# kthohr/mcmc

Hardware: AMD Instinct MI355X
Metric: leapfrog-steps/sec (chains*dims*steps/s), HMC d=128 correlated Gaussian, 65536 chains (higher is better)
Workload: dtype f64

## Files before the change

include/mi_mcmc_engine/det_math.hpp:

```cpp
#pragma once

#include <hip/hip_runtime.h>
#include <stdint.h>

#define MI_HD __host__ __device__ __forceinline__

#if defined(__HIP_DEVICE_COMPILE__)
#define MI_NO_DS_MERGE __attribute__((target("no-load-store-opt")))
#else
#define MI_NO_DS_MERGE
#endif

namespace mi {

#ifndef MI_KC_MODE
#define MI_KC_MODE 1
#endif
#if defined(__HIP_DEVICE_COMPILE__) && MI_KC_MODE == 1
__device__ __forceinline__ double mi_kc(double c) { asm volatile("" : "+s"(c)); return c; }
#define MI_KC(c) ::mi::mi_kc(c)
#define MI_KCD(c, dep) ::mi::mi_kc(c)
#elif defined(__HIP_DEVICE_COMPILE__) && MI_KC_MODE == 2
template <uint64_t BITS>
__device__ __forceinline__ double mi_kc()
{
    uint32_t lo, hi;
    asm volatile("s_mov_b32 %0, %2\n\ts_mov_b32 %1, %3" : "=s"(lo), "=s"(hi) : "n"((uint32_t)BITS), "n"((uint32_t)(BITS >> 32)));
    return __builtin_bit_cast(double, ((uint64_t)hi << 32) | (uint64_t)lo);
}
template <uint64_t BITS>
__device__ __forceinline__ double mi_kcd(double dep)
{
    uint32_t lo, hi;
    asm volatile("s_mov_b32 %0, %2\n\ts_mov_b32 %1, %3" : "=s"(lo), "=s"(hi) : "n"((uint32_t)BITS), "n"((uint32_t)(BITS >> 32)), "v"(dep));
    return __builtin_bit_cast(double, ((uint64_t)hi << 32) | (uint64_t)lo);
}
#define MI_KC(c) (::mi::mi_kc<__builtin_bit_cast(uint64_t, (double)(c))>())
#define MI_KCD(c, dep) (::mi::mi_kcd<__builtin_bit_cast(uint64_t, (double)(c))>(dep))
#else
#define MI_KC(c) (c)
#define MI_KCD(c, dep) (c)
#endif


MI_HD uint64_t d2u(double x) { return __builtin_bit_cast(uint64_t, x); }
MI_HD double u2d(uint64_t u) { return __builtin_bit_cast(double, u); }
MI_HD double pow2i(int k) { return u2d((uint64_t)(k + 1023) << 52); }
MI_HD double dfma(double a, double b, double c) { return __builtin_fma(a, b, c); }
MI_HD bool is_finite(double x) { return (d2u(x) & 0x7ff0000000000000ULL) != 0x7ff0000000000000ULL; }

constexpr double LN2_HI = 0x1.62e42fee00000p-1;
constexpr double LN2_LO = 0x1.a39ef35793c76p-33;
constexpr double INV_LN2 = 0x1.71547652b82fep+0;
constexpr double PI_4 = 0x1.921fb54442d18p-1;
constexpr double INF = __builtin_huge_val();

MI_HD double det_exp(double x)
{
    if (x != x) return x;
    if (x > 709.782712893384) return INF;
    if (x < -745.2) return 0.0;
    const double kf = __builtin_rint(x * INV_LN2);
    const int k = (int)kf;
    double r = dfma(-kf, LN2_HI, x);
    r = dfma(-kf, LN2_LO, r);
    double p = MI_KCD(1.0 / 87178291200.0, r);
    p = dfma(p, r, MI_KCD(1.0 / 6227020800.0, p));
    p = dfma(p, r, MI_KCD(1.0 / 479001600.0, p));
    p = dfma(p, r, MI_KCD(1.0 / 39916800.0, p));
    p = dfma(p, r, MI_KCD(1.0 / 3628800.0, p));
    p = dfma(p, r, MI_KCD(1.0 / 362880.0, p));
    p = dfma(p, r, MI_KCD(1.0 / 40320.0, p));
    p = dfma(p, r, MI_KCD(1.0 / 5040.0, p));
    p = dfma(p, r, MI_KCD(1.0 / 720.0, p));
    p = dfma(p, r, MI_KCD(1.0 / 120.0, p));
    p = dfma(p, r, MI_KCD(1.0 / 24.0, p));
    p = dfma(p, r, MI_KCD(1.0 / 6.0, p));
    p = dfma(p, r, 0.5);
    p = dfma(p, r, 1.0);
    p = dfma(p, r, 1.0);
    const int k1 = k / 2, k2 = k - k1;
    return (p * pow2i(k1)) * pow2i(k2);
// ... 226 lines not shown
```

include/mi_mcmc_engine/hmc_dense.hpp:

```cpp
#pragma once

#include "det_math.hpp"

#ifndef MI_HMC_RNG_STAGED
#define MI_HMC_RNG_STAGED 0
#endif

#ifndef MI_HMC_RNG_PAIRS
#define MI_HMC_RNG_PAIRS 1
#endif

#ifndef MI_HMC_WPB
#define MI_HMC_WPB 8
#endif

namespace mi {

typedef double double4_t __attribute__((ext_vector_type(4)));

struct HmcParams {
    const double* P;
    uint32_t d;
    uint64_t C;
    uint64_t chain0;
// ... 190 lines not shown
            if (v != v) return (ub - lb) / 2;
            return (v < 0.0) ? lb + EPS_DBL : ub - EPS_DBL;
        }
        const double e = det_exp(v);
        const double r = (lb - EPS_DBL + (ub + EPS_DBL) * e) / (1.0 + e);
        return is_finite(r) ? r : ub - EPS_DBL;
    }
    default: return v;
    }
}
__device__ MI_BOX_INLINE double box_inv_jacobian(double v, int bt, double lb, double ub)
{
    switch (bt) {
    case 2: return det_exp(-v);
    case 3: return det_exp(v);
    case 4: { const double e = det_exp(v); return ((e + 1) * (e + 1)) / (e * (ub - lb)); }
    default: return 1.0;
    }
}
__device__ MI_BOX_INLINE double box_log_jacobian_term(double v, int bt, double lb, double ub)
{
    switch (bt) {
    case 2: return v;
    case 3: return -v;
    case 4: {
        const double e = det_exp(v);
        if (is_finite(e)) return det_log(ub - lb) + v - 2 * det_log(1 + e);
        return det_log(ub - lb) - v;
    }
    default: return 0.0;
    }
}

template <int NT, int WPB, bool BOUNDED = false, bool DENSE_M = false, bool DIAGM = false, bool PCM = false>
__global__ MI_NO_DS_MERGE __launch_bounds__(64 * WPB, WPB / 4) void hmc_gauss_mfma_kernel(const HmcParams prm)
{
    static_assert(!PCM || DIAGM, "per-chain masses ride the diagonal-mass variant");
    static_assert(!DENSE_M || BOUNDED, "the dense preconditioner rides the general variant");
    static_assert(!DIAGM || !BOUNDED, "DIAGM is the plain kernel with a diagonal mass; bounds take the general variant");
    constexpr int NS = 4 * NT;
    extern __shared__ __attribute__((aligned(16))) double lds_P[];
    stage_precision<NT>(prm.P, prm.d, lds_P);
    double* lds_lb = lds_P + NT * NS * 64;
    double* lds_ub = lds_lb + 16 * NT;
    double* lds_ms = lds_ub + 16 * NT;
    double* lds_mi = lds_ms + 16 * NT;
    int* lds_bt = reinterpret_cast<int*>(lds_mi + 16 * NT);
    double* lds_Minv = lds_mi + 16 * NT + 8 * NT;
    double* lds_L = lds_Minv + NT * NS * 64;
    if constexpr (DENSE_M && !dense_m_from_global<NT>()) {
        stage_precision<NT>(prm.Minv, prm.d, lds_Minv);
        stage_precision<NT>(prm.Lchol, prm.d, lds_L);
    }
    if (BOUNDED) {
        for (int i = threadIdx.x; i < 16 * NT; i += blockDim.x) {
            const bool in = (uint32_t)i < prm.d;
            lds_lb[i] = in ? prm.lb[i] : 0.0;
            lds_ub[i] = in ? prm.ub[i] : 0.0;
            lds_bt[i] = in ? prm.btype[i] : 1;
            lds_ms[i] = in ? prm.m_sqrt[i] : 1.0;
            lds_mi[i] = in ? prm.m_inv[i] : 1.0;
        }
        __syncthreads();
    }
    if (DIAGM && !PCM) {
        for (int i = threadIdx.x; i < 16 * NT; i += blockDim.x) {
            const bool in = (uint32_t)i < prm.d;
            lds_ms[i] = in ? prm.m_sqrt[i] : 1.0;
            lds_mi[i] = in ? prm.m_inv[i] : 1.0;
        }
        __syncthreads();
    }

    const int lane = threadIdx.x & 63, wave = threadIdx.x >> 6;
    const int j = lane >> 4;
    uint32_t bslices = 0;
    if constexpr (BOUNDED) {
        if (prm.vals_bound)
            for (int s_ = 0; s_ < 4 * NT; ++s_) {
                const bool any = lds_bt[4 * s_] != 1 || lds_bt[4 * s_ + 1] != 1 || lds_bt[4 * s_ + 2] != 1 || lds_bt[4 * s_ + 3] != 1;
                bslices |= (any ? 1u : 0u) << s_;
            }
        bslices = (uint32_t)__builtin_amdgcn_readfirstlane((int)bslices);
    }
    auto slice_bounded = [&](int s) -> bool { return ((bslices >> s) & 1u) != 0u; };
    [[maybe_unused]] auto mi_col = [&]() __attribute__((always_inline)) -> const double* {
        const double* p = lds_mi + (lane >> 4);
        asm volatile("" : "+v"(p));
        return p;
    };
    const uint64_t cl = ((uint64_t)blockIdx.x * WPB + wave) * 16 + (lane & 15);
    const bool live = cl < prm.C;
    const uint64_t cld = live ? cl : prm.C - 1;
    [[maybe_unused]] auto pcm_at = [&](const double* tab, int s) __attribute__((always_inline)) -> double {
        uint32_t dim = 4u * (uint32_t)s + (uint32_t)(lane >> 4);
        asm volatile("" : "+v"(dim));
        return tab[(size_t)(dim < prm.d ? dim : 0u) * prm.C + cld];
    };
    auto minv_at = [&]([[maybe_unused]] const double* mic, int s) __attribute__((always_inline)) -> double {
        if constexpr (PCM) return pcm_at(prm.m_inv, s); else return mic[4 * s];
    };
    const uint64_t chain = prm.chain0 + cl;
    const uint32_t d = prm.d;
    const uint64_t C = prm.C;
    const double eps = prm.eps;
    const double* afrag = lds_P + lane;
    [[maybe_unused]] const double* afrag_minv = (DENSE_M && dense_m_from_global<NT>()) ? prm.Minv + lane : lds_Minv + lane;
    [[maybe_unused]] const double* afrag_l = (DENSE_M && dense_m_from_global<NT>()) ? prm.Lchol + lane : lds_L + lane;

    double th[NS], pm[NS], w[NS];
    double xs[BOUNDED ? NS : 1];
    const size_t lane_off = (size_t)j * C + cld;
    double* const ws_wave = prm.wsave + ((size_t)blockIdx.x * WPB + wave) * ((size_t)3 * NS * 64) + lane;
    auto ws_group = [&](int k) -> double* {
        double* b = ws_wave + (size_t)(k & ~7) * 64;
        asm volatile("" : "+v"(b));
        return b + (k & 7) * 64;
    };
    auto th_mem = [&](int s) -> double* { return ws_group(s); };
    auto w_mem = [&](int s) -> double* { return ws_group(NS + s); };
    [[maybe_unused]] auto z_mem = [&](int s) -> double* { return ws_wave + (size_t)(2 * NS + s) * 64; };

    auto gradient = [&]() __attribute__((always_inline)) {
        if constexpr (BOUNDED) {
#pragma unroll
            for (int s = 0; s < NS; ++s) {
                const int i = 4 * s + j;
                if (slice_bounded(s)) xs[s] = ((uint32_t)i < d) ? box_inv_transform(th[s], lds_bt[i], lds_lb[i], lds_ub[i]) : 0.0;
                else xs[s] = ((uint32_t)i < d) ? th[s] : 0.0;
            }
            target_times<NT>(afrag, prm.P, d, prm.sep_target != 0u, xs, w);
        } else {
            matvec_mfma<NT>(afrag, th, w);
        }
    };
    auto kick_terms = [&](double (&t)[BOUNDED ? NS : 1]) __attribute__((always_inline)) {
        if constexpr (BOUNDED) {
#pragma unroll
            for (int s = 0; s < NS; ++s) {
                const int i = 4 * s + j;
                if (slice_bounded(s)) t[s] = box_inv_jacobian(th[s], lds_bt[i], lds_lb[i], lds_ub[i]) * w[s];
                else t[s] = 1.0 * w[s];
            }
            if (prm.vals_bound) dense_product_poison<NS>(w, t, j, d);
#pragma unroll
            for (int s = 0; s < NS; ++s) t[s] = (eps * t[s]) / 2.0;
        }
    };
    auto kinetic = [&]() __attribute__((always_inline)) -> double {
        if constexpr (BOUNDED) {
            double mp[NS];
            if constexpr (DENSE_M) {
                matvec_m2<NT>(afrag_minv, pm, mp);
            } else {
#pragma unroll
                for (int s = 0; s < NS; ++s) mp[s] = lds_mi[4 * s + j] * pm[s];
                dense_product_poison<NS>(pm, mp, j, d);
            }
            double q = 0.0;
#pragma unroll
            for (int s = 0; s < NS; ++s) q = dfma(pm[s], mp[s], q);
            q = q + __shfl_xor(q, 32);
            q = q + __shfl_xor(q, 16);
            return q / 2.0;
        } else if constexpr (DIAGM) {
            double q = 0.0;
            const double* mic = PCM ? nullptr : mi_col();
#pragma unroll
            for (int s = 0; s < NS; ++s) q = dfma(pm[s], minv_at(mic, s) * pm[s], q);
            q = q + __shfl_xor(q, 32);
            q = q + __shfl_xor(q, 16);
            return q / 2.0;
        } else {
            return dot4<NS>(pm, pm) / 2.0;
        }
    };
    auto potential = [&]() __attribute__((always_inline)) -> double {
        if constexpr (BOUNDED) {
            const double kval = -0.5 * dot4<NS>(xs, w);
            double lj = 0.0;
#pragma unroll
            for (int s = 0; s < NS; ++s) {
                if (!slice_bounded(s)) continue;
                const int i0 = 4 * s;
                const int bt = lds_bt[4 * s + j];
                const double term = box_log_jacobian_term(th[s], bt, lds_lb[4 * s + j], lds_ub[4 * s + j]);
#pragma unroll
                for (int g = 0; g < 4; ++g) {
                    const double tg = __shfl(term, (lane & 15) + 16 * g);
                    if ((uint32_t)(i0 + g) < d && lds_bt[i0 + g] != 1) lj = lj + tg;
                }
            }
            return -(kval + lj);
        } else {
            return 0.5 * dot4<NS>(th, w);
        }
    };

#pragma unroll
    for (int s = 0; s < NS; ++s) {
        const uint32_t dim = 4 * s + j;
        const double v = prm.theta[(size_t)(dim < d ? dim : 0u) * C + cld];
        if constexpr (BOUNDED) th[s] = (dim < d) ? box_transform(v, lds_bt[dim], lds_lb[dim], lds_ub[dim]) : 0.0;
        else th[s] = (dim < d) ? v : 0.0;
    }
    gradient();
    if (live) {
#pragma unroll
        for (int s = 0; s < NS; ++s) { *th_mem(s) = th[s]; *w_mem(s) = w[s]; }
    }
    double prev_U = potential();
    uint64_t n_acc = 0;
    const uint32_t n_total = prm.n_burnin + prm.n_keep;
    [[maybe_unused]] bool nf_seen = false;

    if (WPB > 4 && wave >= 4)
        for (uint32_t k = 0; k < prm.stagger; ++k) __builtin_amdgcn_s_sleep(127);

    const unsigned long long t_loop0 = clock64();
#pragma unroll 1
    for (uint32_t draw = 0; draw < n_total; ++draw) {
#if MI_HMC_RNG_STAGED
#pragma unroll 1
        for (int b = 0; b < NS / 2; ++b) {
            double z0, z1;
            if (prm.ablate & 4u) { z0 = 0.25; z1 = -0.5; }
            else rng_normal_pair_at(prm.seed, chain, draw + prm.draw0, (uint32_t)(4 * b), (uint32_t)j, STREAM_NORMAL, z0, z1);
            *z_mem(2 * b) = (8u * b + j < d) ? z0 : 0.0;
            *z_mem(2 * b + 1) = (8u * b + 4 + j < d) ? z1 : 0.0;
        }
#pragma unroll
        for (int s = 0; s < NS; ++s) pm[s] = *z_mem(s);
        if constexpr (DENSE_M) {
            double zz[NS];
#pragma unroll
            for (int s = 0; s < NS; ++s) zz[s] = pm[s];
            matvec_m2<NT>(afrag_l, zz, pm);
        } else if constexpr (BOUNDED || DIAGM) {
#pragma unroll
            for (int s = 0; s < NS; ++s) pm[s] = lds_ms[4 * s + j] * pm[s];
        }
#else
#pragma unroll
        for (int b = 0; b < NS / 2; ++b) {
            double z0, z1;
            if (prm.ablate & 4u) { z0 = 0.25; z1 = -0.5; }
            else rng_normal_pair_at(prm.seed, chain, draw + prm.draw0, (uint32_t)(4 * b), (uint32_t)j, STREAM_NORMAL, z0, z1);
            pm[2 * b] = (8u * b + j < d) ? z0 : 0.0;
            pm[2 * b + 1] = (8u * b + 4 + j < d) ? z1 : 0.0;
            if constexpr (DIAGM && PCM) {
                pm[2 * b] = pcm_at(prm.m_sqrt, 2 * b) * pm[2 * b];
                pm[2 * b + 1] = pcm_at(prm.m_sqrt, 2 * b + 1) * pm[2 * b + 1];
            } else if constexpr (DIAGM) {
                const double* msc = lds_ms + (lane >> 4);
                asm volatile("" : "+v"(msc));
                pm[2 * b] = msc[8 * b] * pm[2 * b];
                pm[2 * b + 1] = msc[8 * b + 4] * pm[2 * b + 1];
            } else if constexpr (BOUNDED && !DENSE_M) {
                pm[2 * b] = lds_ms[8 * b + j] * pm[2 * b];
                pm[2 * b + 1] = lds_ms[8 * b + 4 + j] * pm[2 * b + 1];
            }
            if (BOUNDED || MI_HMC_RNG_PAIRS == 1 || (b & 1)) __builtin_amdgcn_sched_barrier(0);
        }
        if constexpr (DENSE_M) {
            double zz[NS];
#pragma unroll
            for (int s = 0; s < NS; ++s) zz[s] = pm[s];
            matvec_m2<NT>(afrag_l, zz, pm);
        }
#endif
        const double prev_K = kinetic();

        if constexpr (!BOUNDED) {
            const uint32_t L = prm.n_leap_steps;
            if (L > 0 && (prm.ablate & 3u) != 1u) {
                [[maybe_unused]] const double* mic = (DIAGM && !PCM) ? mi_col() : nullptr;
#pragma unroll
                for (int s = 0; s < NS; ++s) {
                    pm[s] = pm[s] - (eps * w[s]) / 2.0;
                    if constexpr (DIAGM) th[s] = th[s] + eps * (minv_at(mic, s) * pm[s]);
                    else th[s] = th[s] + eps * pm[s];
                }
            }
#pragma unroll 1
            for (uint32_t k = 0; k + 1 < L; ++k) {
                if ((prm.ablate & 3u) != 2u) gradient();
                if ((prm.ablate & 3u) != 1u) {
                    [[maybe_unused]] const double* mic = (DIAGM && !PCM) ? mi_col() : nullptr;
#pragma unroll
                    for (int s = 0; s < NS; ++s) {
                        const double t = (eps * w[s]) / 2.0;
                        pm[s] = pm[s] - t;
                        pm[s] = pm[s] - t;
                        if constexpr (DIAGM) th[s] = th[s] + eps * (minv_at(mic, s) * pm[s]);
                        else th[s] = th[s] + eps * pm[s];
                    }
                }
            }
            if (L > 0) {
                if ((prm.ablate & 3u) != 2u) gradient();
                if ((prm.ablate & 3u) != 1u) {
#pragma unroll
                    for (int s = 0; s < NS; ++s) pm[s] = pm[s] - (eps * w[s]) / 2.0;
                }
            }
        } else {
            const uint32_t L = prm.n_leap_steps;
            auto drift_step = [&]() __attribute__((always_inline)) {
                double mp[NS];
                if constexpr (DENSE_M) {
                    matvec_m2<NT>(afrag_minv, pm, mp);
                } else {
#pragma unroll
                    for (int s = 0; s < NS; ++s) mp[s] = lds_mi[4 * s + j] * pm[s];
                    dense_product_poison<NS>(pm, mp, j, d);
                }
#pragma unroll
                for (int s = 0; s < NS; ++s) th[s] = th[s] + eps * mp[s];
            };
            if (L > 0) {
                double t[NS];
                kick_terms(t);
#pragma unroll
                for (int s = 0; s < NS; ++s) pm[s] = pm[s] - t[s];
                drift_step();
            }
#pragma unroll 1
            for (uint32_t k = 0; k + 1 < L; ++k) {
                gradient();
                double t[NS];
                kick_terms(t);
#pragma unroll
                for (int s = 0; s < NS; ++s) {
                    pm[s] = pm[s] - t[s];
                    pm[s] = pm[s] - t[s];
                }
                drift_step();
            }
            if (L > 0) {
                gradient();
                double t[NS];
                kick_terms(t);
#pragma unroll
                for (int s = 0; s < NS; ++s) pm[s] = pm[s] - t[s];
            }
        }
        if constexpr (BOUNDED) { if (prm.n_leap_steps == 0) gradient(); }

        double prop_U = potential();
        const bool u_nf = !is_finite(prop_U);
        if (u_nf) prop_U = INF;
        const double prop_K = kinetic();
        if constexpr (!BOUNDED) nf_seen |= u_nf | !is_finite(prop_K);
        const double x = -(prop_U + prop_K) + (prev_U + prev_K);
        const double comp_val = (x < 0.01) ? x : 0.01;
        const double z = rng_uniform(prm.seed, chain, draw + prm.draw0, 0u);
        const bool accept = z < det_exp(comp_val);
#ifndef MI_HMC_NO_WSAVE
#define MI_HMC_NO_WSAVE 0
#endif
        if constexpr (MI_HMC_NO_WSAVE && !BOUNDED) {
            if (accept) {
                prev_U = prop_U;
                if (live && !(prm.ablate & 8u)) {
#pragma unroll
                    for (int s = 0; s < NS; ++s) *th_mem(s) = th[s];
                }
            }
            if (__ballot(!accept) != 0ull) {
                if (!accept) {
#pragma unroll
                    for (int s = 0; s < NS; ++s) th[s] = *th_mem(s);
                }
                gradient();
            }
        } else
        if (accept) {
            prev_U = prop_U;
            if (live && !(prm.ablate & 8u)) {
#pragma unroll
                for (int s = 0; s < NS; ++s) { *th_mem(s) = th[s]; *w_mem(s) = w[s]; }
            }
        } else {
#pragma unroll
            for (int s = 0; s < NS; ++s) { th[s] = *th_mem(s); w[s] = *w_mem(s); }
        }
        if (draw >= prm.n_burnin) {
            n_acc += accept ? 1u : 0u;
            if (prm.draws != nullptr && live && !(prm.ablate & 16u)) {
                double* out = prm.draws + (size_t)(draw - prm.n_burnin) * d * C;
#pragma unroll
                for (int s = 0; s < NS; ++s) {
                    const uint32_t dim = 4 * s + j;
                    if (dim < d) (out + (size_t)(4 * s) * C)[lane_off] =
                        (BOUNDED && slice_bounded(s)) ? box_inv_transform(th[s], lds_bt[dim], lds_lb[dim], lds_ub[dim]) : th[s];
                }
            }
        }
    }

    bool replay = false;
    if constexpr (!BOUNDED) replay = nf_seen && prm.nf_flag != nullptr;
    if (live && replay && j == 0) { prm.nf_flag[cl] = 1u; prm.nf_flag[C] = 1u; }
    if (live && !replay) {
#pragma unroll
        for (int s = 0; s < NS; ++s) {
            const uint32_t dim = 4 * s + j;
            if (dim < d) prm.theta[(size_t)dim * C + cl] =
                (BOUNDED && slice_bounded(s)) ? box_inv_transform(th[s], lds_bt[dim], lds_lb[dim], lds_ub[dim]) : th[s];
        }
    }
    if (live && !replay && j == 0) {
        if (prm.n_accept) prm.n_accept[cl] = n_acc;
        if (prm.n_leap) prm.n_leap[cl] = (prm.ablate & 32u) ? (uint64_t)(clock64() - t_loop0)
                                                            : (uint64_t)n_total * prm.n_leap_steps;
    }
}

}
```

include/mi_mcmc_engine/tile_samplers.hpp:

```cpp
#pragma once

#include <type_traits>

#include "hmc_dense.hpp"

namespace mi {

struct TileParams {
    uint32_t d;
    uint64_t C, chain0;
    double* theta;
    double* wsave;
    double* draws;
    uint64_t* n_accept;
    uint64_t* n_leap;
    uint64_t seed;
    uint32_t n_burnin, n_keep, n_leap_steps, draw0;
    double eps;
    double s2, rs, cons_term, log_det;
    double* ws;
    double* step_out;
    uint32_t* depth_trace;
    double* adapt_state;
    uint32_t n_adapt, max_depth;
// ... 194 lines not shown
        const double v = prm.theta[(size_t)(dim < d ? dim : 0u) * C + cld];
        th[s] = (dim < d) ? v : 0.0;
    }
    tgt.grad_tile(lds_t, th, g, val, true);
    if (live) {
#pragma unroll
        for (int s = 0; s < NS; ++s) { *ws_group(s) = th[s]; *ws_group(NS + s) = g[s]; }
    }
    double prev_U = -val;
    uint64_t n_acc = 0;
    const uint32_t n_total = prm.n_burnin + prm.n_keep;
    const uint32_t L = prm.n_leap_steps;
    auto kinetic = [&]() __attribute__((always_inline)) -> double {
        return diag_quadratic<NS>(pm, 1.0, j, d) / 2.0;
    };
    auto drift = [&]() __attribute__((always_inline)) {
#pragma unroll
        for (int s = 0; s < NS; ++s) th[s] = th[s] + eps * pm[s];
        dense_product_poison<NS>(pm, th, j, d);
    };
#pragma unroll 1
    for (uint32_t draw = 0; draw < n_total; ++draw) {
#pragma unroll
        for (int b = 0; b < NS / 2; ++b) {
            double z0, z1;
            rng_normal_pair_at(prm.seed, chain, draw + prm.draw0, (uint32_t)(4 * b), (uint32_t)j, STREAM_NORMAL, z0, z1);
            pm[2 * b] = (8u * b + j < d) ? z0 : 0.0;
            pm[2 * b + 1] = (8u * b + 4 + j < d) ? z1 : 0.0;
            __builtin_amdgcn_sched_barrier(0);
        }
        const double prev_K = kinetic();
        if (L > 0) {
#pragma unroll
            for (int s = 0; s < NS; ++s) pm[s] = pm[s] + (eps * g[s]) / 2.0;
            drift();
        }
#pragma unroll 1
        for (uint32_t k = 0; k + 1 < L; ++k) {
            double unused;
            tgt.grad_tile(lds_t, th, g, unused, false);
#pragma unroll
            for (int s = 0; s < NS; ++s) {
                const double t = (eps * g[s]) / 2.0;
                pm[s] = pm[s] + t;
                pm[s] = pm[s] + t;
            }
            drift();
        }
        if (L > 0) {
            tgt.grad_tile(lds_t, th, g, val, true);
#pragma unroll
            for (int s = 0; s < NS; ++s) pm[s] = pm[s] + (eps * g[s]) / 2.0;
        }
        double prop_U = -val;
        if (!is_finite(prop_U)) prop_U = INF;
        const double prop_K = kinetic();
        const double x = -(prop_U + prop_K) + (prev_U + prev_K);
        const double comp_val = (x < 0.01) ? x : 0.01;
        const double z = rng_uniform(prm.seed, chain, draw + prm.draw0, 0u);
        const bool accept = z < det_exp(comp_val);
        if (accept) {
            prev_U = prop_U;
            if (live) {
#pragma unroll
                for (int s = 0; s < NS; ++s) { *ws_group(s) = th[s]; *ws_group(NS + s) = g[s]; }
            }
        } else {
#pragma unroll
            for (int s = 0; s < NS; ++s) { th[s] = *ws_group(s); g[s] = *ws_group(NS + s); }
            val = -prev_U;
        }
        if (draw >= prm.n_burnin) {
            n_acc += accept ? 1u : 0u;
            if (prm.draws != nullptr && live) {
                double* out = prm.draws + (size_t)(draw - prm.n_burnin) * d * C;
#pragma unroll
                for (int s = 0; s < NS; ++s) {
                    const uint32_t dim = 4 * s + j;
                    if (dim < d) (out + (size_t)(4 * s) * C)[lane_off] = th[s];
                }
            }
        }
    }
    if (live) {
#pragma unroll
// ... 263 lines not shown
```

mcmc_amd/csrc/hmc_diag.hpp:

```cpp
#pragma once

#include "det_math.hpp"

namespace mi {

struct HmcDiagParams {
    const double* prec;
    uint32_t d;
    uint64_t C, chain0;
    double* theta;
    double* scratch;
    double* draws;
    uint64_t* n_accept;
    uint64_t* n_leap;
    uint64_t seed;
    uint32_t n_burnin, n_keep, n_leap_steps;
    double eps;
    uint32_t draw0;
    const double* m_sqrt;
    const double* m_inv;
    uint32_t m_per_chain;
    uint32_t* nf_flag;
};

// ... 46 lines not shown
        }
        prev_U = 0.5 * diag_combine(q);
    }
    uint64_t n_acc = 0;
    const uint32_t n_total = prm.n_burnin + prm.n_keep;
    uint32_t pp = 0;
    bool nf_seen = false;

    for (uint32_t draw = 0; draw < n_total; ++draw) {
        const bool kept = draw >= prm.n_burnin;
        double* dst = (kept && prm.draws) ? prm.draws + (size_t)(draw - prm.n_burnin) * slab + c
                                          : prm.scratch + (size_t)pp * slab + c;
        if (dst == cur) { pp ^= 1u; dst = prm.scratch + (size_t)pp * slab + c; }
        double qk0 = 0.0, qu1 = 0.0, qk1 = 0.0;
        for (uint32_t b = 0; b * 8 < d; b += TR / 2) {
            double z[TR], th[TR], pm[TR], lam[TR], w[TR], mi_[PRECOND ? TR : 1];
            rng_normal_pair(prm.seed, chain, draw + prm.draw0, 4 * b + j, STREAM_NORMAL, z[0], z[1]);
            if constexpr (TR == 4) rng_normal_pair(prm.seed, chain, draw + prm.draw0, 4 * (b + 1) + j, STREAM_NORMAL, z[TR - 2], z[TR - 1]);
#pragma unroll
            for (int r = 0; r < TR; ++r) {
                const uint32_t i = 8 * b + 4 * (uint32_t)r + j;
                const uint32_t ic = i < d ? i : d - 1;
                th[r] = cur[(size_t)ic * C];
                lam[r] = prec ? prec[ic] : 1.0;
                if constexpr (PRECOND) { pm[r] = msq[(size_t)ic * mstr] * z[r]; mi_[r] = miv[(size_t)ic * mstr]; }
                else pm[r] = z[r];
                w[r] = lam[r] * th[r];
            }
#pragma unroll
            for (int r = 0; r < TR; ++r)
                if (8 * b + 4 * (uint32_t)r + j < d) qk0 = dfma(pm[r], PRECOND ? mi_[PRECOND ? r : 0] * pm[r] : pm[r], qk0);
            if (L > 0) {
#pragma unroll
                for (int r = 0; r < TR; ++r) pm[r] = pm[r] - (eps * w[r]) / 2.0;
            }
            for (uint32_t kk = (uint32_t)__builtin_amdgcn_readfirstlane((int)((L > 0) ? L - 1 : 0u)); kk != 0u; kk = (uint32_t)__builtin_amdgcn_readfirstlane((int)(kk - 1u))) {
#pragma unroll
                for (int r = 0; r < TR; ++r) {
                    if constexpr (PRECOND) th[r] = th[r] + eps * (mi_[PRECOND ? r : 0] * pm[r]);
                    else th[r] = th[r] + eps * pm[r];
                    w[r] = lam[r] * th[r];
                    const double t = (eps * w[r]) / 2.0;
                    pm[r] = pm[r] - t;
                    pm[r] = pm[r] - t;
                }
            }
            if (L > 0) {
#pragma unroll
                for (int r = 0; r < TR; ++r) {
                    if constexpr (PRECOND) th[r] = th[r] + eps * (mi_[PRECOND ? r : 0] * pm[r]);
                    else th[r] = th[r] + eps * pm[r];
                    w[r] = lam[r] * th[r];
                    pm[r] = pm[r] - (eps * w[r]) / 2.0;
                }
            }
#pragma unroll
            for (int r = 0; r < TR; ++r) {
                const uint32_t i = 8 * b + 4 * (uint32_t)r + j;
                if (i < d) {
                    qu1 = dfma(th[r], w[r], qu1);
                    qk1 = dfma(pm[r], PRECOND ? mi_[PRECOND ? r : 0] * pm[r] : pm[r], qk1);
                    if (live) dst[(size_t)i * C] = th[r];
                }
            }
        }
        const double prev_K = diag_combine(qk0) / 2.0;
        double prop_U = 0.5 * diag_combine(qu1);
        const bool u_nf = !is_finite(prop_U);
        if (u_nf) prop_U = INF;
        const double prop_K = diag_combine(qk1) / 2.0;
        nf_seen |= u_nf | !is_finite(prop_K);
        const double x = -(prop_U + prop_K) + (prev_U + prev_K);
        const double comp_val = (x < 0.01) ? x : 0.01;
        const double zu = rng_uniform(prm.seed, chain, draw + prm.draw0, 0u);
        const bool accept = zu < det_exp(comp_val);
        if (accept) {
            cur = dst;
            prev_U = prop_U;
            if (!(kept && prm.draws)) pp ^= 1u;
        } else if (kept && prm.draws) {
            if (live)
                for (uint32_t i = j; i < d; i += 4) dst[(size_t)i * C] = cur[(size_t)i * C];
            cur = dst;
        }
        if (kept) n_acc += accept ? 1u : 0u;
    }
// ... 38 lines not shown
            q[i & 3] = dfma(t, w, q[i & 3]);
        }
        prev_U = 0.5 * ((q[0] + q[2]) + (q[1] + q[3]));
    }
    uint64_t n_acc = 0;
    const uint32_t n_total = prm.n_burnin + prm.n_keep;
    uint32_t pp = 0;
    bool nf_seen = false;

    for (uint32_t draw = 0; draw < n_total; ++draw) {
        const bool kept = draw >= prm.n_burnin;
        double* dst = (kept && prm.draws) ? prm.draws + (size_t)(draw - prm.n_burnin) * slab + c
                                          : prm.scratch + (size_t)pp * slab + c;
        if (dst == cur) { pp ^= 1u; dst = prm.scratch + (size_t)pp * slab + c; }
        double qk0[4] = {0, 0, 0, 0}, qu1[4] = {0, 0, 0, 0}, qk1[4] = {0, 0, 0, 0};
        for (uint32_t b = 0; b * 8 < d; ++b) {
            double z[8], th[8], pm[8], lam[8], w[8], mi_[PRECOND ? 8 : 1];
#pragma unroll
            for (int j = 0; j < 4; ++j) rng_normal_pair(prm.seed, chain, draw + prm.draw0, 4 * b + j, STREAM_NORMAL, z[j], z[4 + j]);
#pragma unroll
            for (int r = 0; r < 8; ++r) {
                const uint32_t i = 8 * b + r;
                const uint32_t ic = i < d ? i : d - 1;
                th[r] = cur[(size_t)ic * C];
                lam[r] = prec ? prec[ic] : 1.0;
                if constexpr (PRECOND) { pm[r] = msq[(size_t)ic * mstr] * z[r]; mi_[r] = miv[(size_t)ic * mstr]; }
                else pm[r] = z[r];
                w[r] = lam[r] * th[r];
            }
#pragma unroll
            for (int r = 0; r < 8; ++r) if (8 * b + r < d) qk0[r & 3] = dfma(pm[r], PRECOND ? mi_[PRECOND ? r : 0] * pm[r] : pm[r], qk0[r & 3]);
            if (L > 0) {
#pragma unroll
                for (int r = 0; r < 8; ++r) pm[r] = pm[r] - (eps * w[r]) / 2.0;
            }
            for (uint32_t k = 0; k + 1 < L; ++k) {
#pragma unroll
                for (int r = 0; r < 8; ++r) {
                    if constexpr (PRECOND) th[r] = th[r] + eps * (mi_[PRECOND ? r : 0] * pm[r]);
                    else th[r] = th[r] + eps * pm[r];
                    w[r] = lam[r] * th[r];
                    const double t = (eps * w[r]) / 2.0;
                    pm[r] = pm[r] - t;
                    pm[r] = pm[r] - t;
                }
            }
            if (L > 0) {
#pragma unroll
                for (int r = 0; r < 8; ++r) {
                    if constexpr (PRECOND) th[r] = th[r] + eps * (mi_[PRECOND ? r : 0] * pm[r]);
                    else th[r] = th[r] + eps * pm[r];
                    w[r] = lam[r] * th[r];
                    pm[r] = pm[r] - (eps * w[r]) / 2.0;
                }
            }
#pragma unroll
            for (int r = 0; r < 8; ++r) {
                const uint32_t i = 8 * b + r;
                if (i < d) {
                    qu1[r & 3] = dfma(th[r], w[r], qu1[r & 3]);
                    qk1[r & 3] = dfma(pm[r], PRECOND ? mi_[PRECOND ? r : 0] * pm[r] : pm[r], qk1[r & 3]);
                    dst[(size_t)i * C] = th[r];
                }
            }
        }
        const double prev_K = ((qk0[0] + qk0[2]) + (qk0[1] + qk0[3])) / 2.0;
        double prop_U = 0.5 * ((qu1[0] + qu1[2]) + (qu1[1] + qu1[3]));
        const bool u_nf = !is_finite(prop_U);
        if (u_nf) prop_U = INF;
        const double prop_K = ((qk1[0] + qk1[2]) + (qk1[1] + qk1[3])) / 2.0;
        nf_seen |= u_nf | !is_finite(prop_K);
        const double x = -(prop_U + prop_K) + (prev_U + prev_K);
        const double comp_val = (x < 0.01) ? x : 0.01;
        const double zu = rng_uniform(prm.seed, chain, draw + prm.draw0, 0u);
        const bool accept = zu < det_exp(comp_val);
        if (accept) {
            cur = dst;
            prev_U = prop_U;
            if (!(kept && prm.draws)) pp ^= 1u;
        } else if (kept && prm.draws) {
            for (uint32_t i = 0; i < d; ++i) dst[(size_t)i * C] = cur[(size_t)i * C];
            cur = dst;
        }
        if (kept) n_acc += accept ? 1u : 0u;
    }
    if (nf_seen && prm.nf_flag != nullptr) { prm.nf_flag[c] = 1u; prm.nf_flag[C] = 1u; return; }
// ... 11 lines not shown
```

mcmc_amd/csrc/hmc_launch.hip:

```cpp
#include "hmc_dense.hpp"
#include "hmc_split.hpp"
#include "launchers.hpp"
#include "launch_common.hpp"

namespace mi {
namespace {

template <int NT>
int plain(const HmcParams& prm, hipStream_t st)
{
    constexpr int WPB = MI_HMC_WPB;
    const size_t lds = (size_t)NT * 4 * NT * 64 * sizeof(double);
    auto kern = hmc_gauss_mfma_kernel<NT, WPB>;
    MI_LAUNCH_TRY(hipFuncSetAttribute(reinterpret_cast<const void*>(kern), hipFuncAttributeMaxDynamicSharedMemorySize, (int)lds));
    const unsigned grid = (unsigned)((prm.C + 16 * WPB - 1) / (16 * WPB));
    note_kernel("hmc_gauss_mfma_kernel<%d, %d, false, false, false>", NT, WPB);
    hipLaunchKernelGGL(kern, dim3(grid), dim3(64 * WPB), lds, st, prm);
    return (int)hipGetLastError();
}

template <int NT, bool PCM = false>
int plain_diagm(const HmcParams& prm, hipStream_t st)
{
    constexpr int WPB = MI_HMC_WPB;
    const size_t lds = (size_t)NT * 4 * NT * 64 * sizeof(double) + (size_t)16 * NT * (4 * sizeof(double) + sizeof(int));
    auto kern = hmc_gauss_mfma_kernel<NT, WPB, false, false, true, PCM>;
    MI_LAUNCH_TRY(hipFuncSetAttribute(reinterpret_cast<const void*>(kern), hipFuncAttributeMaxDynamicSharedMemorySize, (int)lds));
    const unsigned grid = (unsigned)((prm.C + 16 * WPB - 1) / (16 * WPB));
    note_kernel("hmc_gauss_mfma_kernel<%d, %d, false, false, true%s>", NT, WPB, PCM ? ", true" : "");
    hipLaunchKernelGGL(kern, dim3(grid), dim3(64 * WPB), lds, st, prm);
    return (int)hipGetLastError();
}

template <int NT>
int plain4(const HmcParams& prm, hipStream_t st)
{
    const size_t lds = (size_t)NT * 4 * NT * 64 * sizeof(double);
    auto kern = hmc_gauss_mfma_kernel<NT, 4>;
    MI_LAUNCH_TRY(hipFuncSetAttribute(reinterpret_cast<const void*>(kern), hipFuncAttributeMaxDynamicSharedMemorySize, (int)lds));
    note_kernel("hmc_gauss_mfma_kernel<%d, 4, false, false, false>", NT);
    hipLaunchKernelGGL(kern, dim3((unsigned)((prm.C + 63) / 64)), dim3(256), lds, st, prm);
    return (int)hipGetLastError();
}

template <int NT, int SPLIT, int WPB>
int split(const HmcParams& prm, hipStream_t st)
{
    const size_t lds = hmc_split_lds_bytes<NT, SPLIT, WPB>();
    int dev = 0, lds_max = 0;
    MI_LAUNCH_TRY(hipGetDevice(&dev));
    MI_LAUNCH_TRY(hipDeviceGetAttribute(&lds_max, hipDeviceAttributeMaxSharedMemoryPerBlock, dev));
    if ((size_t)lds_max < lds) return (int)hipErrorInvalidValue;
    auto kern = hmc_gauss_split_kernel<NT, SPLIT, WPB>;
    MI_LAUNCH_TRY(hipFuncSetAttribute(reinterpret_cast<const void*>(kern), hipFuncAttributeMaxDynamicSharedMemorySize, (int)lds));
    const unsigned chains_per_wg = 16 * (WPB / SPLIT);
    note_kernel("hmc_gauss_split_kernel<%d, %d, %d>", NT, SPLIT, WPB);
    hipLaunchKernelGGL(kern, dim3((unsigned)((prm.C + chains_per_wg - 1) / chains_per_wg)), dim3(64 * WPB), lds, st, prm);
    return (int)hipGetLastError();
}

}

int launch_hmc_gauss(const HmcParams& prm, int nt, bool gen, bool dense_m, hipStream_t st)
{
    if (dense_m) return launch_hmc_gauss_dense_m(prm, nt, st);
    if (gen) return launch_hmc_gauss_general(prm, nt, st);
    return MI_DISPATCH_NT(nt, plain<1>(prm, st), plain<2>(prm, st), plain<4>(prm, st), plain<8>(prm, st));
}

int launch_hmc_gauss_diagm(const HmcParams& prm, int nt, hipStream_t st)
{
// ... 12 lines not shown
```

mcmc_amd/csrc/hmc_split.hpp:

```cpp
#pragma once

#include "hmc_dense.hpp"

namespace mi {

template <int NT, int SPLIT, int WPB = 4>
constexpr size_t hmc_split_lds_bytes()
{
    constexpr int NS = 4 * NT, TILES = WPB / SPLIT;
    return ((size_t)NT * NS * 64 + (size_t)TILES * NS * 64) * sizeof(double);
}

template <int NT, int SPLIT, int WPB>
__device__ __forceinline__ void hmc_split_body(const HmcParams& prm, double* lds_P, const int h)
{
    constexpr int NS = 4 * NT;
    constexpr int NSO = NS / SPLIT;
    constexpr int NTO = NT / SPLIT;
    constexpr int TILES = WPB / SPLIT;
    double* const lds_x = lds_P + NT * NS * 64;

    const int lane = threadIdx.x & 63, wave = threadIdx.x >> 6;
    const int tile = wave / SPLIT;
    const int j = lane >> 4;
// ... 82 lines not shown

#pragma unroll
    for (int k = 0; k < NSO; ++k) {
        const uint32_t dim = 4 * (s0 + k) + j;
        const double v = prm.theta[(size_t)(dim < d ? dim : 0u) * C + cld];
        own[k] = (dim < d) ? v : 0.0;
    }
    gradient();
    if (live) {
#pragma unroll
        for (int k = 0; k < NSO; ++k) { *th_mem(k) = own[k]; *w_mem(k) = w[k]; }
    }
    double prev_U = potential();
    uint64_t n_acc = 0;
    const uint32_t n_total = prm.n_burnin + prm.n_keep;
    const uint32_t L = prm.n_leap_steps;
    bool nf_seen = false;

#pragma unroll 1
    for (uint32_t draw = 0; draw < n_total; ++draw) {
#pragma unroll
        for (int b = 0; b < NSO / 2; ++b) {
            const int bb = s0 / 2 + b;
            double z0, z1;
            rng_normal_pair_at(prm.seed, chain, draw + prm.draw0, (uint32_t)(4 * bb), (uint32_t)j, STREAM_NORMAL, z0, z1);
            pm[2 * b] = (8u * bb + j < d) ? z0 : 0.0;
            pm[2 * b + 1] = (8u * bb + 4 + j < d) ? z1 : 0.0;
            __builtin_amdgcn_sched_barrier(0);
        }
        const double prev_K = kinetic();
        if (L > 0) {
#pragma unroll
            for (int k = 0; k < NSO; ++k) {
                pm[k] = pm[k] - (eps * w[k]) / 2.0;
                own[k] = own[k] + eps * pm[k];
            }
        }
#pragma unroll 1
        for (uint32_t st = 0; st + 1 < L; ++st) {
            gradient();
#pragma unroll
            for (int k = 0; k < NSO; ++k) {
                const double t = (eps * w[k]) / 2.0;
                pm[k] = pm[k] - t;
                pm[k] = pm[k] - t;
                own[k] = own[k] + eps * pm[k];
            }
        }
        if (L > 0) {
            gradient();
#pragma unroll
            for (int k = 0; k < NSO; ++k) pm[k] = pm[k] - (eps * w[k]) / 2.0;
        }
        double prop_U = potential();
        const bool u_nf = !is_finite(prop_U);
        if (u_nf) prop_U = INF;
        const double prop_K = kinetic();
        nf_seen |= u_nf | !is_finite(prop_K);
        const double x = -(prop_U + prop_K) + (prev_U + prev_K);
        const double comp_val = (x < 0.01) ? x : 0.01;
        const double z = rng_uniform(prm.seed, chain, draw + prm.draw0, 0u);
        const bool accept = z < det_exp(comp_val);
        if (accept) {
            prev_U = prop_U;
            if (live) {
#pragma unroll
                for (int k = 0; k < NSO; ++k) { *th_mem(k) = own[k]; *w_mem(k) = w[k]; }
            }
        } else {
#pragma unroll
            for (int k = 0; k < NSO; ++k) { own[k] = *th_mem(k); w[k] = *w_mem(k); }
        }
        if (draw >= prm.n_burnin) {
            n_acc += accept ? 1u : 0u;
            if (prm.draws != nullptr && live) {
                double* out = prm.draws + (size_t)(draw - prm.n_burnin) * d * C;
#pragma unroll
                for (int k = 0; k < NSO; ++k) {
                    const uint32_t dim = 4 * (s0 + k) + j;
                    if (dim < d) (out + (size_t)(4 * (s0 + k)) * C)[lane_off] = own[k];
                }
            }
        }
    }

// ... 29 lines not shown
```

Baseline: 265.9 billion.

## Add full-tile kernel instantiation and fuse half-kick scaling into FMA

Adds a FULL template variant, chosen when d equals 16*NT, that drops the per-dimension bounds checks and writes draws and theta through a running pointer with a fixed stride. It also replaces (eps*w)/2 subtracted from p with a single fma by -0.5 on eps*w, which removes the divide and separate subtract in every leapfrog kick. State save and restore are grouped per 8-slice block to cut address arithmetic. The fma form rounds differently from the old two-step expression, so bitwise results may change, and the extra instantiation adds to code size.

```diff
diff --git a/include/mi_mcmc_engine/det_math.hpp b/include/mi_mcmc_engine/det_math.hpp
--- a/include/mi_mcmc_engine/det_math.hpp
+++ b/include/mi_mcmc_engine/det_math.hpp
@@ -48,6 +48,8 @@
 MI_HD double pow2i(int k) { return u2d((uint64_t)(k + 1023) << 52); }
 MI_HD double dfma(double a, double b, double c) { return __builtin_fma(a, b, c); }
 MI_HD bool is_finite(double x) { return (d2u(x) & 0x7ff0000000000000ULL) != 0x7ff0000000000000ULL; }
+
+MI_HD double half_kick(double p, double t1, int sign) { return __builtin_fma(sign < 0 ? -0.5 : 0.5, t1, p); }
 
 constexpr double LN2_HI = 0x1.62e42fee00000p-1;
 constexpr double LN2_LO = 0x1.a39ef35793c76p-33;
diff --git a/include/mi_mcmc_engine/hmc_dense.hpp b/include/mi_mcmc_engine/hmc_dense.hpp
--- a/include/mi_mcmc_engine/hmc_dense.hpp
+++ b/include/mi_mcmc_engine/hmc_dense.hpp
@@ -246,12 +246,13 @@
     }
 }
 
-template <int NT, int WPB, bool BOUNDED = false, bool DENSE_M = false, bool DIAGM = false, bool PCM = false>
+template <int NT, int WPB, bool BOUNDED = false, bool DENSE_M = false, bool DIAGM = false, bool PCM = false, bool FULL = false>
 __global__ MI_NO_DS_MERGE __launch_bounds__(64 * WPB, WPB / 4) void hmc_gauss_mfma_kernel(const HmcParams prm)
 {
     static_assert(!PCM || DIAGM, "per-chain masses ride the diagonal-mass variant");
     static_assert(!DENSE_M || BOUNDED, "the dense preconditioner rides the general variant");
     static_assert(!DIAGM || !BOUNDED, "DIAGM is the plain kernel with a diagonal mass; bounds take the general variant");
+    static_assert(!FULL || !BOUNDED, "the full-tile instantiation is for the plain and DIAGM variants");
     constexpr int NS = 4 * NT;
     extern __shared__ __attribute__((aligned(16))) double lds_P[];
     stage_precision<NT>(prm.P, prm.d, lds_P);
@@ -309,7 +310,7 @@
     [[maybe_unused]] auto pcm_at = [&](const double* tab, int s) __attribute__((always_inline)) -> double {
         uint32_t dim = 4u * (uint32_t)s + (uint32_t)(lane >> 4);
         asm volatile("" : "+v"(dim));
-        return tab[(size_t)(dim < prm.d ? dim : 0u) * prm.C + cld];
+        return tab[(size_t)((FULL || dim < prm.d) ? dim : 0u) * prm.C + cld];
     };
     auto minv_at = [&]([[maybe_unused]] const double* mic, int s) __attribute__((always_inline)) -> double {
         if constexpr (PCM) return pcm_at(prm.m_inv, s); else return mic[4 * s];
@@ -318,6 +319,7 @@
     const uint32_t d = prm.d;
     const uint64_t C = prm.C;
     const double eps = prm.eps;
+    auto in_d = [&](uint32_t dim) __attribute__((always_inline)) -> bool { return FULL || dim < d; };
     const double* afrag = lds_P + lane;
     [[maybe_unused]] const double* afrag_minv = (DENSE_M && dense_m_from_global<NT>()) ? prm.Minv + lane : lds_Minv + lane;
     [[maybe_unused]] const double* afrag_l = (DENSE_M && dense_m_from_global<NT>()) ? prm.Lchol + lane : lds_L + lane;
@@ -331,8 +333,17 @@
         asm volatile("" : "+v"(b));
         return b + (k & 7) * 64;
     };
-    auto th_mem = [&](int s) -> double* { return ws_group(s); };
-    auto w_mem = [&](int s) -> double* { return ws_group(NS + s); };
+    constexpr int WG = NS < 8 ? NS : 8;
+    auto save_state = [&]() __attribute__((always_inline)) {
+#pragma unroll
+        for (int g = 0; g < NS; g += WG) {
+            double* const tb = ws_group(g);
+            double* const wb = ws_group(NS + g);
+#pragma unroll
+            for (int i = 0; i < WG; ++i) { tb[i * 64] = th[g + i]; wb[i * 64] = w[g + i]; }
+        }
+    };
+    [[maybe_unused]] auto th_mem = [&](int s) -> double* { return ws_group(s); };
     [[maybe_unused]] auto z_mem = [&](int s) -> double* { return ws_wave + (size_t)(2 * NS + s) * 64; };
 
     auto gradient = [&]() __attribute__((always_inline)) {
@@ -358,7 +369,7 @@
             }
             if (prm.vals_bound) dense_product_poison<NS>(w, t, j, d);
 #pragma unroll
-            for (int s = 0; s < NS; ++s) t[s] = (eps * t[s]) / 2.0;
+            for (int s = 0; s < NS; ++s) t[s] = eps * t[s];
         }
     };
     auto kinetic = [&]() __attribute__((always_inline)) -> double {
@@ -414,15 +425,12 @@
 #pragma unroll
     for (int s = 0; s < NS; ++s) {
         const uint32_t dim = 4 * s + j;
-        const double v = prm.theta[(size_t)(dim < d ? dim : 0u) * C + cld];
+        const double v = prm.theta[(size_t)(in_d(dim) ? dim : 0u) * C + cld];
         if constexpr (BOUNDED) th[s] = (dim < d) ? box_transform(v, lds_bt[dim], lds_lb[dim], lds_ub[dim]) : 0.0;
-        else th[s] = (dim < d) ? v : 0.0;
+        else th[s] = in_d(dim) ? v : 0.0;
     }
     gradient();
-    if (live) {
-#pragma unroll
-        for (int s = 0; s < NS; ++s) { *th_mem(s) = th[s]; *w_mem(s) = w[s]; }
-    }
+    if (live) save_state();
     double prev_U = potential();
     uint64_t n_acc = 0;
     const uint32_t n_total = prm.n_burnin + prm.n_keep;
@@ -440,8 +448,8 @@
             double z0, z1;
             if (prm.ablate & 4u) { z0 = 0.25; z1 = -0.5; }
             else rng_normal_pair_at(prm.seed, chain, draw + prm.draw0, (uint32_t)(4 * b), (uint32_t)j, STREAM_NORMAL, z0, z1);
-            *z_mem(2 * b) = (8u * b + j < d) ? z0 : 0.0;
-            *z_mem(2 * b + 1) = (8u * b + 4 + j < d) ? z1 : 0.0;
+            *z_mem(2 * b) = in_d(8u * b + j) ? z0 : 0.0;
+            *z_mem(2 * b + 1) = in_d(8u * b + 4 + j) ? z1 : 0.0;
         }
 #pragma unroll
         for (int s = 0; s < NS; ++s) pm[s] = *z_mem(s);
@@ -460,8 +468,8 @@
             double z0, z1;
             if (prm.ablate & 4u) { z0 = 0.25; z1 = -0.5; }
             else rng_normal_pair_at(prm.seed, chain, draw + prm.draw0, (uint32_t)(4 * b), (uint32_t)j, STREAM_NORMAL, z0, z1);
-            pm[2 * b] = (8u * b + j < d) ? z0 : 0.0;
-            pm[2 * b + 1] = (8u * b + 4 + j < d) ? z1 : 0.0;
+            pm[2 * b] = in_d(8u * b + j) ? z0 : 0.0;
+            pm[2 * b + 1] = in_d(8u * b + 4 + j) ? z1 : 0.0;
             if constexpr (DIAGM && PCM) {
                 pm[2 * b] = pcm_at(prm.m_sqrt, 2 * b) * pm[2 * b];
                 pm[2 * b + 1] = pcm_at(prm.m_sqrt, 2 * b + 1) * pm[2 * b + 1];
@@ -491,7 +499,7 @@
                 [[maybe_unused]] const double* mic = (DIAGM && !PCM) ? mi_col() : nullptr;
 #pragma unroll
                 for (int s = 0; s < NS; ++s) {
-                    pm[s] = pm[s] - (eps * w[s]) / 2.0;
+                    pm[s] = half_kick(pm[s], eps * w[s], -1);
                     if constexpr (DIAGM) th[s] = th[s] + eps * (minv_at(mic, s) * pm[s]);
                     else th[s] = th[s] + eps * pm[s];
                 }
@@ -503,9 +511,9 @@
                     [[maybe_unused]] const double* mic = (DIAGM && !PCM) ? mi_col() : nullptr;
 #pragma unroll
                     for (int s = 0; s < NS; ++s) {
-                        const double t = (eps * w[s]) / 2.0;
-                        pm[s] = pm[s] - t;
-                        pm[s] = pm[s] - t;
+                        const double t1 = eps * w[s];
+                        pm[s] = half_kick(pm[s], t1, -1);
+                        pm[s] = half_kick(pm[s], t1, -1);
                         if constexpr (DIAGM) th[s] = th[s] + eps * (minv_at(mic, s) * pm[s]);
                         else th[s] = th[s] + eps * pm[s];
                     }
@@ -515,7 +523,7 @@
                 if ((prm.ablate & 3u) != 2u) gradient();
                 if ((prm.ablate & 3u) != 1u) {
 #pragma unroll
-                    for (int s = 0; s < NS; ++s) pm[s] = pm[s] - (eps * w[s]) / 2.0;
+                    for (int s = 0; s < NS; ++s) pm[s] = half_kick(pm[s], eps * w[s], -1);
                 }
             }
         } else {
@@ -536,7 +544,7 @@
                 double t[NS];
                 kick_terms(t);
 #pragma unroll
-                for (int s = 0; s < NS; ++s) pm[s] = pm[s] - t[s];
+                for (int s = 0; s < NS; ++s) pm[s] = half_kick(pm[s], t[s], -1);
                 drift_step();
             }
 #pragma unroll 1
@@ -546,8 +554,8 @@
                 kick_terms(t);
 #pragma unroll
                 for (int s = 0; s < NS; ++s) {
-                    pm[s] = pm[s] - t[s];
-                    pm[s] = pm[s] - t[s];
+                    pm[s] = half_kick(pm[s], t[s], -1);
+                    pm[s] = half_kick(pm[s], t[s], -1);
                 }
                 drift_step();
             }
@@ -556,7 +564,7 @@
                 double t[NS];
                 kick_terms(t);
 #pragma unroll
-                for (int s = 0; s < NS; ++s) pm[s] = pm[s] - t[s];
+                for (int s = 0; s < NS; ++s) pm[s] = half_kick(pm[s], t[s], -1);
             }
         }
         if constexpr (BOUNDED) { if (prm.n_leap_steps == 0) gradient(); }
@@ -591,23 +599,40 @@
         } else
         if (accept) {
             prev_U = prop_U;
-            if (live && !(prm.ablate & 8u)) {
-#pragma unroll
-                for (int s = 0; s < NS; ++s) { *th_mem(s) = th[s]; *w_mem(s) = w[s]; }
-            }
+            if (live && !(prm.ablate & 8u)) save_state();
         } else {
 #pragma unroll
-            for (int s = 0; s < NS; ++s) { th[s] = *th_mem(s); w[s] = *w_mem(s); }
+            for (int g = 0; g < NS; g += WG) {
+                const double* const tb = ws_group(g);
+                const double* const wb = ws_group(NS + g);
+#pragma unroll
+                for (int i = 0; i < WG; ++i) {
+                    th[g + i] = tb[i * 64];
+                    w[g + i] = wb[i * 64];
+                    __builtin_amdgcn_sched_barrier(0);
+                }
+            }
         }
         if (draw >= prm.n_burnin) {
             n_acc += accept ? 1u : 0u;
             if (prm.draws != nullptr && live && !(prm.ablate & 16u)) {
                 double* out = prm.draws + (size_t)(draw - prm.n_burnin) * d * C;
-#pragma unroll
-                for (int s = 0; s < NS; ++s) {
-                    const uint32_t dim = 4 * s + j;
-                    if (dim < d) (out + (size_t)(4 * s) * C)[lane_off] =
-                        (BOUNDED && slice_bounded(s)) ? box_inv_transform(th[s], lds_bt[dim], lds_lb[dim], lds_ub[dim]) : th[s];
+                if constexpr (FULL) {
+                    double* o = out + lane_off;
+                    const size_t row4 = (size_t)4 * C;
+#pragma unroll
+                    for (int s = 0; s < NS; ++s) {
+                        *o = th[s];
+                        o += row4;
+                        asm volatile("" : "+v"(o));
+                    }
+                } else {
+#pragma unroll
+                    for (int s = 0; s < NS; ++s) {
+                        const uint32_t dim = 4 * s + j;
+                        if (dim < d) (out + (size_t)(4 * s) * C)[lane_off] =
+                            (BOUNDED && slice_bounded(s)) ? box_inv_transform(th[s], lds_bt[dim], lds_lb[dim], lds_ub[dim]) : th[s];
+                    }
                 }
             }
         }
@@ -617,11 +642,23 @@
     if constexpr (!BOUNDED) replay = nf_seen && prm.nf_flag != nullptr;
     if (live && replay && j == 0) { prm.nf_flag[cl] = 1u; prm.nf_flag[C] = 1u; }
     if (live && !replay) {
-#pragma unroll
-        for (int s = 0; s < NS; ++s) {
-            const uint32_t dim = 4 * s + j;
-            if (dim < d) prm.theta[(size_t)dim * C + cl] =
-                (BOUNDED && slice_bounded(s)) ? box_inv_transform(th[s], lds_bt[dim], lds_lb[dim], lds_ub[dim]) : th[s];
+        if constexpr (FULL) {
+            double* o = prm.theta + lane_off;
+            asm volatile("" : "+v"(o));
+            const size_t row4 = (size_t)4 * C;
+#pragma unroll
+            for (int s = 0; s < NS; ++s) {
+                *o = th[s];
+                o += row4;
+                asm volatile("" : "+v"(o));
+            }
+        } else {
+#pragma unroll
+            for (int s = 0; s < NS; ++s) {
+                const uint32_t dim = 4 * s + j;
+                if (dim < d) prm.theta[(size_t)dim * C + cl] =
+                    (BOUNDED && slice_bounded(s)) ? box_inv_transform(th[s], lds_bt[dim], lds_lb[dim], lds_ub[dim]) : th[s];
+            }
         }
     }
     if (live && !replay && j == 0) {
diff --git a/include/mi_mcmc_engine/tile_samplers.hpp b/include/mi_mcmc_engine/tile_samplers.hpp
--- a/include/mi_mcmc_engine/tile_samplers.hpp
+++ b/include/mi_mcmc_engine/tile_samplers.hpp
@@ -250,7 +250,7 @@
         const double prev_K = kinetic();
         if (L > 0) {
 #pragma unroll
-            for (int s = 0; s < NS; ++s) pm[s] = pm[s] + (eps * g[s]) / 2.0;
+            for (int s = 0; s < NS; ++s) pm[s] = half_kick(pm[s], eps * g[s], +1);
             drift();
         }
 #pragma unroll 1
@@ -259,16 +259,16 @@
             tgt.grad_tile(lds_t, th, g, unused, false);
 #pragma unroll
             for (int s = 0; s < NS; ++s) {
-                const double t = (eps * g[s]) / 2.0;
-                pm[s] = pm[s] + t;
-                pm[s] = pm[s] + t;
+                const double t1 = eps * g[s];
+                pm[s] = half_kick(pm[s], t1, +1);
+                pm[s] = half_kick(pm[s], t1, +1);
             }
             drift();
         }
         if (L > 0) {
             tgt.grad_tile(lds_t, th, g, val, true);
 #pragma unroll
-            for (int s = 0; s < NS; ++s) pm[s] = pm[s] + (eps * g[s]) / 2.0;
+            for (int s = 0; s < NS; ++s) pm[s] = half_kick(pm[s], eps * g[s], +1);
         }
         double prop_U = -val;
         if (!is_finite(prop_U)) prop_U = INF;
diff --git a/mcmc_amd/csrc/hmc_diag.hpp b/mcmc_amd/csrc/hmc_diag.hpp
--- a/mcmc_amd/csrc/hmc_diag.hpp
+++ b/mcmc_amd/csrc/hmc_diag.hpp
@@ -102,7 +102,7 @@
                 if (8 * b + 4 * (uint32_t)r + j < d) qk0 = dfma(pm[r], PRECOND ? mi_[PRECOND ? r : 0] * pm[r] : pm[r], qk0);
             if (L > 0) {
 #pragma unroll
-                for (int r = 0; r < TR; ++r) pm[r] = pm[r] - (eps * w[r]) / 2.0;
+                for (int r = 0; r < TR; ++r) pm[r] = half_kick(pm[r], eps * w[r], -1);
             }
             for (uint32_t kk = (uint32_t)__builtin_amdgcn_readfirstlane((int)((L > 0) ? L - 1 : 0u)); kk != 0u; kk = (uint32_t)__builtin_amdgcn_readfirstlane((int)(kk - 1u))) {
 #pragma unroll
@@ -110,9 +110,9 @@
                     if constexpr (PRECOND) th[r] = th[r] + eps * (mi_[PRECOND ? r : 0] * pm[r]);
                     else th[r] = th[r] + eps * pm[r];
                     w[r] = lam[r] * th[r];
-                    const double t = (eps * w[r]) / 2.0;
-                    pm[r] = pm[r] - t;
-                    pm[r] = pm[r] - t;
+                    const double t1 = eps * w[r];
+                    pm[r] = half_kick(pm[r], t1, -1);
+                    pm[r] = half_kick(pm[r], t1, -1);
                 }
             }
             if (L > 0) {
@@ -121,7 +121,7 @@
                     if constexpr (PRECOND) th[r] = th[r] + eps * (mi_[PRECOND ? r : 0] * pm[r]);
                     else th[r] = th[r] + eps * pm[r];
                     w[r] = lam[r] * th[r];
-                    pm[r] = pm[r] - (eps * w[r]) / 2.0;
+                    pm[r] = half_kick(pm[r], eps * w[r], -1);
                 }
             }
 #pragma unroll
@@ -226,7 +226,7 @@
             for (int r = 0; r < 8; ++r) if (8 * b + r < d) qk0[r & 3] = dfma(pm[r], PRECOND ? mi_[PRECOND ? r : 0] * pm[r] : pm[r], qk0[r & 3]);
             if (L > 0) {
 #pragma unroll
-                for (int r = 0; r < 8; ++r) pm[r] = pm[r] - (eps * w[r]) / 2.0;
+                for (int r = 0; r < 8; ++r) pm[r] = half_kick(pm[r], eps * w[r], -1);
             }
             for (uint32_t k = 0; k + 1 < L; ++k) {
 #pragma unroll
@@ -234,9 +234,9 @@
                     if constexpr (PRECOND) th[r] = th[r] + eps * (mi_[PRECOND ? r : 0] * pm[r]);
                     else th[r] = th[r] + eps * pm[r];
                     w[r] = lam[r] * th[r];
-                    const double t = (eps * w[r]) / 2.0;
-                    pm[r] = pm[r] - t;
-                    pm[r] = pm[r] - t;
+                    const double t1 = eps * w[r];
+                    pm[r] = half_kick(pm[r], t1, -1);
+                    pm[r] = half_kick(pm[r], t1, -1);
                 }
             }
             if (L > 0) {
@@ -245,7 +245,7 @@
                     if constexpr (PRECOND) th[r] = th[r] + eps * (mi_[PRECOND ? r : 0] * pm[r]);
                     else th[r] = th[r] + eps * pm[r];
                     w[r] = lam[r] * th[r];
-                    pm[r] = pm[r] - (eps * w[r]) / 2.0;
+                    pm[r] = half_kick(pm[r], eps * w[r], -1);
                 }
             }
 #pragma unroll
diff --git a/mcmc_amd/csrc/hmc_launch.hip b/mcmc_amd/csrc/hmc_launch.hip
--- a/mcmc_amd/csrc/hmc_launch.hip
+++ b/mcmc_amd/csrc/hmc_launch.hip
@@ -11,7 +11,7 @@
 {
     constexpr int WPB = MI_HMC_WPB;
     const size_t lds = (size_t)NT * 4 * NT * 64 * sizeof(double);
-    auto kern = hmc_gauss_mfma_kernel<NT, WPB>;
+    auto kern = prm.d == 16u * NT ? hmc_gauss_mfma_kernel<NT, WPB, false, false, false, false, true> : hmc_gauss_mfma_kernel<NT, WPB>;
     MI_LAUNCH_TRY(hipFuncSetAttribute(reinterpret_cast<const void*>(kern), hipFuncAttributeMaxDynamicSharedMemorySize, (int)lds));
     const unsigned grid = (unsigned)((prm.C + 16 * WPB - 1) / (16 * WPB));
     note_kernel("hmc_gauss_mfma_kernel<%d, %d, false, false, false>", NT, WPB);
@@ -24,7 +24,7 @@
 {
     constexpr int WPB = MI_HMC_WPB;
     const size_t lds = (size_t)NT * 4 * NT * 64 * sizeof(double) + (size_t)16 * NT * (4 * sizeof(double) + sizeof(int));
-    auto kern = hmc_gauss_mfma_kernel<NT, WPB, false, false, true, PCM>;
+    auto kern = prm.d == 16u * NT ? hmc_gauss_mfma_kernel<NT, WPB, false, false, true, PCM, true> : hmc_gauss_mfma_kernel<NT, WPB, false, false, true, PCM>;
     MI_LAUNCH_TRY(hipFuncSetAttribute(reinterpret_cast<const void*>(kern), hipFuncAttributeMaxDynamicSharedMemorySize, (int)lds));
     const unsigned grid = (unsigned)((prm.C + 16 * WPB - 1) / (16 * WPB));
     note_kernel("hmc_gauss_mfma_kernel<%d, %d, false, false, true%s>", NT, WPB, PCM ? ", true" : "");
@@ -36,7 +36,7 @@
 int plain4(const HmcParams& prm, hipStream_t st)
 {
     const size_t lds = (size_t)NT * 4 * NT * 64 * sizeof(double);
-    auto kern = hmc_gauss_mfma_kernel<NT, 4>;
+    auto kern = prm.d == 16u * NT ? hmc_gauss_mfma_kernel<NT, 4, false, false, false, false, true> : hmc_gauss_mfma_kernel<NT, 4>;
     MI_LAUNCH_TRY(hipFuncSetAttribute(reinterpret_cast<const void*>(kern), hipFuncAttributeMaxDynamicSharedMemorySize, (int)lds));
     note_kernel("hmc_gauss_mfma_kernel<%d, 4, false, false, false>", NT);
     hipLaunchKernelGGL(kern, dim3((unsigned)((prm.C + 63) / 64)), dim3(256), lds, st, prm);
diff --git a/mcmc_amd/csrc/hmc_split.hpp b/mcmc_amd/csrc/hmc_split.hpp
--- a/mcmc_amd/csrc/hmc_split.hpp
+++ b/mcmc_amd/csrc/hmc_split.hpp
@@ -138,7 +138,7 @@
         if (L > 0) {
 #pragma unroll
             for (int k = 0; k < NSO; ++k) {
-                pm[k] = pm[k] - (eps * w[k]) / 2.0;
+                pm[k] = half_kick(pm[k], eps * w[k], -1);
                 own[k] = own[k] + eps * pm[k];
             }
         }
@@ -147,16 +147,16 @@
             gradient();
 #pragma unroll
             for (int k = 0; k < NSO; ++k) {
-                const double t = (eps * w[k]) / 2.0;
-                pm[k] = pm[k] - t;
-                pm[k] = pm[k] - t;
+                const double t1 = eps * w[k];
+                pm[k] = half_kick(pm[k], t1, -1);
+                pm[k] = half_kick(pm[k], t1, -1);
                 own[k] = own[k] + eps * pm[k];
             }
         }
         if (L > 0) {
             gradient();
 #pragma unroll
-            for (int k = 0; k < NSO; ++k) pm[k] = pm[k] - (eps * w[k]) / 2.0;
+            for (int k = 0; k < NSO; ++k) pm[k] = half_kick(pm[k], eps * w[k], -1);
         }
         double prop_U = potential();
         const bool u_nf = !is_finite(prop_U);
```

After: 267.1 billion, median of 6. About the same (+0.4%).
